# smritip/real-time-audio-sync

Hardware: AMD Instinct MI355X
Metric: aligned chroma frames/sec, batch=64 OTW c=500; path-index match vs CPU ref (higher is better)
Workload: dtype f64 arithmetic, f32 features in HBM

## Files before the change

include/rtsync.h:

```cpp
#ifndef RTSYNC_H
#define RTSYNC_H

#include <stddef.h>
#include <stdint.h>

#ifdef __cplusplus
extern "C" {
#endif

#define RTS_OK 0
#define RTS_ERR_INVALID (-1)
#define RTS_ERR_UNSUPPORTED (-2)
#define RTS_ERR_HIP (-3)
#define RTS_ERR_NO_DEVICE (-4)

#define RTS_F32 0
#define RTS_F64 1
#define RTS_I16 2

#define RTS_VARIANT_OTW 0
#define RTS_VARIANT_LIVENOTE 1
#define RTS_VARIANT_LIVENOTE_V2 2

#define RTS_COST_DOT 0
// ... 15 lines not shown
#define RTS_STATE_LEN 16
#define RTS_ST_T 0
#define RTS_ST_J 1
#define RTS_ST_DIRECTION 2
#define RTS_ST_PREVIOUS 3
#define RTS_ST_RUN_COUNT 4
#define RTS_ST_STATUS 5
#define RTS_ST_FIRST_INSERT 6
#define RTS_ST_N_PATH 7
#define RTS_ST_CONSUMED 8
#define RTS_ST_ROW_STRIPS 9
#define RTS_ST_COL_STRIPS 10
#define RTS_ST_CELLS_LO 11
#define RTS_ST_CELLS_HI 12
#define RTS_ST_PATH_TRUNCATED 13
#define RTS_ST_BAND_RECOMPUTES 15

const char *rts_last_error(void);
int rts_version(void);
int rts_device_count(void);

typedef struct rts_otw rts_otw;

int rts_otw_create(const void *ref_dev, int ref_dtype, int F, int N, int B, int c, int max_run_count,
                   int variant, int cost_kind, rts_otw **out);
int rts_otw_create_refs(const void *refs_dev, int ref_dtype, int F, long long n_ref_frames,
                        const long long *first_host, const int32_t *len_host, int B, int c, int max_run_count,
                        int variant, int cost_kind, rts_otw **out);
int rts_otw_destroy(rts_otw *h);
int rts_otw_reset(rts_otw *h, void *stream);

int rts_otw_restart(rts_otw *h, const uint8_t *mask_host, const long long *first_host, const int32_t *len_host,
                    void *stream);

int rts_otw_run(rts_otw *h, const void *live_dev, int live_dtype, int T_max, const int32_t *live_len_dev,
                int mode, void *stream);

int rts_otw_insert(rts_otw *h, const void *frames_dev, int frames_dtype, const uint8_t *active_dev,
                   void *stream);

int rts_otw_push(rts_otw *h, const void *frames_dev, int frames_dtype, int n_max, const int32_t *n_new_dev,
                 void *stream);

int rts_otw_recent(rts_otw *h, int M_max, double *out_dev , int32_t *len_dev ,
                   const uint8_t *mask_dev , void *stream);

int rts_otw_path_cost(rts_otw *h, int K, double *mean_dev , int32_t *n_dev ,
                      double *costs_dev , void *stream);

int rts_otw_read_state(rts_otw *h, int b, int32_t *state , void *stream);
int rts_otw_read_states(rts_otw *h, int32_t *states , void *stream);
int rts_otw_read_path(rts_otw *h, int b, int32_t *pairs, int cap_pairs, int *n, void *stream);
int rts_otw_read_bands(rts_otw *h, int b, double *row_band, double *col_band, void *stream);
int rts_otw_device_views(rts_otw *h, int32_t **path_dev, int *path_cap, int32_t **state_dev);
int rts_otw_set_dense(rts_otw *h, double *acc_dev, double *cost_dev, void *stream);
int rts_otw_replay_dense(rts_otw *h, const void *live_dev, int live_dtype, int T_max, const int32_t *live_len_dev,
                         double *acc_dev, double *cost_dev, void *stream);
int rts_otw_set_waves(rts_otw *h, int waves);
const char *rts_otw_kernel_name(const rts_otw *h);


int rts_dtw_workspace_bytes(int M, int N, int B, size_t *bytes);

int rts_dtw(const void *a_dev, int a_dtype, long long a_stride, const void *b_dev, int b_dtype,
            long long b_stride, int F, int M, int N, int B, double *cost_dev, double *acc_dev,
            int8_t *back_dev, int32_t *path_dev, int32_t *path_len_dev, void *ws_dev, size_t ws_bytes,
            void *stream);

int rts_dtw_paths_workspace_bytes(int M_max, int N_max, int B, size_t *bytes);

int rts_dtw_paths(const void *a_dev, int a_dtype, long long a_stride, const int32_t *a_len_dev, const void *b_dev,
                  int b_dtype, long long b_stride, const int32_t *b_len_dev, int F, int M_max, int N_max, int B,
                  int32_t *path_dev, int32_t *path_len_dev, double *total_dev, void *ws_dev, size_t ws_bytes,
                  void *stream);

int rts_dtw_subseq_paths_workspace_bytes(int M_max, int N_max, int B, size_t *bytes);

int rts_dtw_subseq_paths(const void *a_dev, int a_dtype, long long a_stride, const int32_t *a_len_dev,
                         const void *b_dev, int b_dtype, long long b_stride, const int32_t *b_len_dev,
                         int F, int M_max, int N_max, int B,
                         int32_t *path_dev, int32_t *path_len_dev, double *total_dev,
                         int32_t *start_dev, int32_t *end_dev, double *row_dev ,
                         void *ws_dev, size_t ws_bytes, void *stream);


int rts_locate(const void *queries_dev, int q_dtype, int M_max, const int32_t *q_len_dev, int B, const void *pool_dev,
               int pool_dtype, int F, long long n_pool_frames, const long long *piece_first_dev,
               const int32_t *piece_len_dev, int P, int cost_kind, double *cost_dev, int32_t *end_dev,
               int32_t *start_dev, double *row_dev, int32_t *rowstart_dev, void *stream);

typedef struct rts_chroma rts_chroma;

long long rts_chroma_num_frames(long long n_samples, int fft_len, int hop, int pad_left);

int rts_chroma_create(int fft_len, int hop, const double *window_host, const double *fb_host, rts_chroma **out);
int rts_chroma_destroy(rts_chroma *h);

int rts_chroma_frames(rts_chroma *h, const void *samples_dev, int sample_dtype, long long n_samples,
                      int pad_left, int n_frames, int normalize, void *chroma_out_dev, int out_dtype,
                      double *stft_out_dev, void *stream);

int rts_chroma_frames_batch(rts_chroma *h, const void *samples_dev, int sample_dtype, long long sample_stride,
                            const int32_t *n_samples_dev, int pad_left, int B, int n_frames_max,
                            const int32_t *n_frames_dev, int normalize, void *chroma_out_dev, int out_dtype,
                            void *stream);

// ... 85 lines not shown
```

real_time_audio_sync_amd/_native.py:

```python
import ctypes
import os

import torch

_HERE = os.path.dirname(os.path.abspath(__file__))
SO_PATH = os.environ.get("RTSYNC_LIB") or os.path.join(_HERE, "librtsync.so")

F32, F64, I16 = 0, 1, 2
VARIANT_OTW, VARIANT_LIVENOTE, VARIANT_LIVENOTE_V2 = 0, 1, 2
COST_DOT, COST_EUCLID = 0, 1
FEATURE_CHROMA, FEATURE_CHROMA_DIFF = 0, 1
DIR_NONE, DIR_BOTH, DIR_ROW, DIR_COLUMN = -1, 0, 1, 2
RUNNING, STOP_REF_END, LIVE_OVERFLOW, DEVICE_FAULT = 0, 1, 2, 3
MODE_INSERT_LOOP, MODE_SET_LIVE = 0, 1
STATE_LEN = 16
(ST_T, ST_J, ST_DIRECTION, ST_PREVIOUS, ST_RUN_COUNT, ST_STATUS, ST_FIRST_INSERT, ST_N_PATH, ST_CONSUMED,
 ST_ROW_STRIPS, ST_COL_STRIPS, ST_CELLS_LO, ST_CELLS_HI, ST_PATH_TRUNCATED) = range(14)
ST_BAND_RECOMPUTES = 15

EXPORTS = {}


class RtsyncError(RuntimeError):
    pass


def _load():
    if not os.path.exists(SO_PATH):
        raise ImportError(
            "librtsync.so is not built (%s). Run `python -c 'import __graft_entry__ as g; g.build()'` "
            "or `python real_time_audio_sync_amd/_build.py`. There is no CPU fallback." % SO_PATH)
    return ctypes.CDLL(SO_PATH)


lib = _load()

_vp, _i32, _pi32 = ctypes.c_void_p, ctypes.c_int, ctypes.POINTER(ctypes.c_int)


def _decl(name, restype, argtypes):
    fn = getattr(lib, name)
    fn.restype = restype
    fn.argtypes = argtypes
    EXPORTS[name] = fn
    return fn


_decl("rts_last_error", ctypes.c_char_p, [])
_decl("rts_version", _i32, [])
_decl("rts_device_count", _i32, [])
_decl("rts_otw_create", _i32, [_vp, _i32, _i32, _i32, _i32, _i32, _i32, _i32, _i32, ctypes.POINTER(_vp)])
_i64 = ctypes.c_longlong
_decl("rts_otw_create_refs", _i32, [_vp, _i32, _i32, _i64, _vp, _vp, _i32, _i32, _i32, _i32, _i32, ctypes.POINTER(_vp)])
_decl("rts_otw_destroy", _i32, [_vp])
_decl("rts_otw_reset", _i32, [_vp, _vp])
_decl("rts_otw_restart", _i32, [_vp, _vp, _vp, _vp, _vp])
_decl("rts_otw_run", _i32, [_vp, _vp, _i32, _i32, _vp, _i32, _vp])
_decl("rts_otw_insert", _i32, [_vp, _vp, _i32, _vp, _vp])
_decl("rts_otw_push", _i32, [_vp, _vp, _i32, _i32, _vp, _vp])
_decl("rts_otw_recent", _i32, [_vp, _i32, _vp, _vp, _vp, _vp])
_decl("rts_otw_path_cost", _i32, [_vp, _i32, _vp, _vp, _vp, _vp])
_decl("rts_otw_read_state", _i32, [_vp, _i32, _vp, _vp])
_decl("rts_otw_read_states", _i32, [_vp, _vp, _vp])
_decl("rts_otw_read_path", _i32, [_vp, _i32, _vp, _i32, _pi32, _vp])
_decl("rts_otw_read_bands", _i32, [_vp, _i32, _vp, _vp, _vp])
_decl("rts_otw_device_views", _i32, [_vp, ctypes.POINTER(_vp), _pi32, ctypes.POINTER(_vp)])
_decl("rts_otw_set_waves", _i32, [_vp, _i32])
_decl("rts_otw_set_dense", _i32, [_vp, _vp, _vp, _vp])
_decl("rts_otw_replay_dense", _i32, [_vp, _vp, _i32, _i32, _vp, _vp, _vp, _vp])
_decl("rts_otw_kernel_name", ctypes.c_char_p, [_vp])
_decl("rts_dtw_workspace_bytes", _i32, [_i32, _i32, _i32, ctypes.POINTER(ctypes.c_size_t)])
_decl("rts_dtw", _i32, [_vp, _i32, _i64, _vp, _i32, _i64, _i32, _i32, _i32, _i32, _vp, _vp, _vp, _vp, _vp, _vp,
                        ctypes.c_size_t, _vp])
_decl("rts_dtw_paths_workspace_bytes", _i32, [_i32, _i32, _i32, ctypes.POINTER(ctypes.c_size_t)])
_decl("rts_dtw_paths", _i32, [_vp, _i32, _i64, _vp, _vp, _i32, _i64, _vp, _i32, _i32, _i32, _i32, _vp, _vp, _vp, _vp,
                              ctypes.c_size_t, _vp])
_decl("rts_dtw_subseq_paths_workspace_bytes", _i32, [_i32, _i32, _i32, ctypes.POINTER(ctypes.c_size_t)])
_decl("rts_dtw_subseq_paths", _i32, [_vp, _i32, _i64, _vp, _vp, _i32, _i64, _vp, _i32, _i32, _i32, _i32, _vp, _vp, _vp, _vp,
                                     _vp, _vp, _vp, ctypes.c_size_t, _vp])
_decl("rts_locate", _i32, [_vp, _i32, _i32, _vp, _i32, _vp, _i32, _i32, _i64, _vp, _vp, _i32, _i32, _vp, _vp, _vp, _vp,
                           _vp, _vp])


_decl("rts_chroma_num_frames", _i64, [_i64, _i32, _i32, _i32])
_decl("rts_chroma_create", _i32, [_i32, _i32, _vp, _vp, ctypes.POINTER(_vp)])
_decl("rts_chroma_destroy", _i32, [_vp])
_decl("rts_chroma_frames", _i32, [_vp, _vp, _i32, _i64, _i32, _i32, _i32, _vp, _i32, _vp, _vp])
_decl("rts_chroma_frames_batch", _i32, [_vp, _vp, _i32, _i64, _vp, _i32, _i32, _i32, _vp, _i32, _vp, _i32, _vp])
_decl("rts_chroma_plan_info", _i32, [_vp, _pi32, _pi32])
_decl("rts_chroma_project", _i32, [_vp, _vp, _i32, _i32, _vp, _i32, _vp])
_decl("rts_chroma_diff", _i32, [_vp, _i32, _i32, _vp, _vp])


_decl("rts_resample_out_len", _i64, [_i64, _i32, _i32])
_decl("rts_resample_avail", _i64, [_i64, _i32, _i32, _i32])
_decl("rts_resample_create", _i32, [_i32, _i32, _vp, _i32, ctypes.POINTER(_vp)])
_decl("rts_resample_destroy", _i32, [_vp])
_decl("rts_resample_run", _i32, [_vp, _vp, _i32, _i64, _vp, _i32, _i32, _vp, _vp, _vp])


_decl("rts_wtw_create", _i32, [_vp, _i32, _i32, _i32, _i32, _i32, _i32, ctypes.POINTER(_vp)])
_decl("rts_wtw_create_refs", _i32, [_vp, _i32, _i64, _vp, _vp, _i32, _i32, _i32, _i32, ctypes.POINTER(_vp)])
_decl("rts_wtw_destroy", _i32, [_vp])
_decl("rts_wtw_reset", _i32, [_vp, _vp])
_decl("rts_wtw_restart", _i32, [_vp, _vp, _vp, _vp, _vp])
_decl("rts_wtw_push", _i32, [_vp, _vp, _i32, _i32, _vp, _i32, _vp])
_decl("rts_wtw_recent", _i32, [_vp, _i32, _vp, _vp, _vp, _vp])
_decl("rts_wtw_read_states", _i32, [_vp, _vp, _vp])
_decl("rts_wtw_read_path", _i32, [_vp, _i32, _vp, _i32, _pi32, _vp])
_decl("rts_wtw_read_last_d", _i32, [_vp, _i32, _vp, _vp])
_decl("rts_wtw_device_views", _i32, [_vp, ctypes.POINTER(_vp), _pi32, ctypes.POINTER(_vp)])
_decl("rts_wtw_state_view", _i32, [_vp, ctypes.POINTER(_vp)])
WTW_STATE_LEN = 8

_decl("rts_live_create", _i32, [_vp, _vp, _vp, _i32, _i32, ctypes.POINTER(_vp)])
_decl("rts_live_create_features", _i32, [_vp, _vp, _vp, _i32, _i32, _i32, ctypes.POINTER(_vp)])
_decl("rts_live_create_resampled", _i32, [_vp, _vp, _vp, _i32, _i32, _i32, _vp, ctypes.POINTER(_vp)])
_decl("rts_live_columns_view", _i32, [_vp, ctypes.POINTER(_vp), _pi32, _pi32, ctypes.POINTER(_vp)])
# ... 43 lines not shown
```

real_time_audio_sync_amd/csrc/otw.hip:

```cpp
#include <hip/hip_runtime.h>
#include <math.h>
#include <stddef.h>
#include <stdint.h>
#include <stdlib.h>
#include <string.h>
#include <type_traits>

#include "common.h"
#include "cost.h"

namespace rts {

constexpr int kF = 12;
constexpr int kFetch = 8;

struct OtwArgs {
    const void *ref;
    const void *live;
    const int32_t *live_len;
    int32_t *state;
    int32_t *path;
    double *bands;
    long long live_stride;
    int N, c, max_run_count, variant, cost_kind, mode;
// ... 2058 lines not shown
    const int32_t *state, *path, *hist_len;
    const double *hist;
    const void *ref;
    const long long *ref_first;
    const int32_t *ref_len;
    int N, path_cap, hist_stride, ref_f64, euclid, K;
    double *mean, *costs;
    int32_t *n_out;
};
__global__ void __launch_bounds__(256) otw_path_cost_kernel(PathCostArgs a) {
    __shared__ double cost_s[256];
    const int b = blockIdx.x, k = threadIdx.x;
    const double qnan = __longlong_as_double(0x7ff8000000000000LL);
    const int Nb = a.ref_len ? a.ref_len[b] : a.N;
    int points = a.state[(size_t)b * RTS_STATE_LEN + RTS_ST_N_PATH];
    points = points > a.path_cap ? a.path_cap : (points < 0 ? 0 : points);
    if (!a.hist) points = 0;
    const int n = points < a.K ? points : a.K;
    int frames = a.hist ? a.hist_len[b] : 0;
    frames = frames > a.hist_stride ? a.hist_stride : frames;
    if (k < a.K) {
        double cost = qnan;
        if (k < n) {
            const int2 p = reinterpret_cast<const int2 *>(a.path)[(size_t)b * a.path_cap + (points - n + k)];
            if (p.x >= 0 && p.x < frames && p.y >= 0 && p.y < Nb) {
                OtwEnv e;
                e.live = a.hist;
                e.live_f64 = 1;
                e.live_base = (long long)b * a.hist_stride * kF;
                e.ref_f64 = a.ref_f64;
                e.ref = a.ref_first ? static_cast<const char *>(a.ref) + a.ref_first[b] * (long long)kF * (a.ref_f64 ? 8 : 4)
                                    : a.ref;
                double lf[kF], rf[kF];
                otw_live_frame(e, p.x, lf);
                otw_ref_frame(e, p.y, rf);
                cost = cell_cost(lf, rf, a.euclid);
            }
        }
        cost_s[k] = cost;
        if (a.costs) a.costs[(size_t)b * a.K + k] = cost;
    }
    __syncthreads();
    if (k == 0) {
        double sum = 0.0;
        for (int i = 0; i < n; i++) sum = sum + cost_s[i];
        a.mean[b] = n > 0 ? sum / (double)n : qnan;
        a.n_out[b] = n;
        __threadfence_system();
    }
}

}

struct rts_otw {
    const void *ref;
    int ref_dtype, F, N, B, c, max_run_count, variant, cost_kind;
    int W, waves, path_cap;
    int hist_stride;
    int32_t *state;
    int32_t *path;
    double *bands;
    double *hist;
    rts::RefTable refs;
    int32_t *hist_len;
    long long *debug;
    double *dense_acc, *dense_cost;
    int spec;
    int device;
    int cus;
    int tp_from;
    const void *attr_fn[8];
    int src_kind;
    int run_dtype, run_T, run_mode;
    int32_t *rp_state, *rp_path;
    double *rp_bands;
};

namespace rts {

static int ensure_lds_attr(rts_otw *h, const void *fn, size_t smem) {
    for (int k = 0; k < 8; k++)
        if (h->attr_fn[k] == fn) return RTS_OK;
    RTS_HIP(hipFuncSetAttribute(fn, hipFuncAttributeMaxDynamicSharedMemorySize, (int)smem));
    for (int k = 0; k < 8; k++)
        if (!h->attr_fn[k]) {
            h->attr_fn[k] = fn;
            break;
        }
    return RTS_OK;
}

template <int W, int NW, bool DENSE, typename RT, bool SPEC>
static int launch_advance_d(rts_otw *h, const OtwArgs &args, int B, hipStream_t s) {
    using LdsT = OtwLds<W, RT>;
    const size_t smem = SPEC ? ((offsetof(LdsT, refw) + 15) & ~(size_t)15) + sizeof(OtwSpecLds<W>)
                             : (kHasLiveRing<RT> ? sizeof(LdsT) : ((offsetof(LdsT, refw) + 15) & ~(size_t)15));
    const int rc = ensure_lds_attr(h, reinterpret_cast<const void *>(&otw_advance_kernel<W, NW, DENSE, RT, SPEC>), smem);
    if (rc != RTS_OK) return rc;
    hipLaunchKernelGGL((otw_advance_kernel<W, NW, DENSE, RT, SPEC>), dim3(B), dim3(64 * NW), smem, s, args);
    RTS_HIP(hipGetLastError());
    return RTS_OK;
}

template <int W, int NW>
static int launch_advance(rts_otw *h, const OtwArgs &args, int B, hipStream_t s) {
    if constexpr (W >= 1024) {
        if (args.dense_acc) return launch_advance_d<W, 8, true, LiveFromGlobal, false>(h, args, B, s);
        if constexpr (NW >= 8) {
            if (args.spec) return launch_advance_d<W, NW, false, LiveFromGlobal, true>(h, args, B, s);
        }
        return set_error(RTS_ERR_UNSUPPORTED, "band widths above 500 (c=%d) run only on the pipelined 8-wave kernel", h->c);
    } else {
        if (args.dense_acc) return launch_advance_d<W, NW, true, double, false>(h, args, B, s);
        const bool f32 = !args.ref_f64 && !args.live_f64;
        if constexpr (NW >= 8) {
            if (args.spec) {
                if (B >= h->tp_from * h->cus && B > 0) return launch_advance_d<W, NW, false, LiveFromGlobalLean, true>(h, args, B, s);
                if (f32) return launch_advance_d<W, NW, false, float, true>(h, args, B, s);
                return (B <= h->cus) ? launch_advance_d<W, NW, false, double, true>(h, args, B, s)
                                     : launch_advance_d<W, NW, false, LiveFromGlobal, true>(h, args, B, s);
            }
        }
        return f32 ? launch_advance_d<W, NW, false, float, false>(h, args, B, s)
                   : launch_advance_d<W, NW, false, double, false>(h, args, B, s);
    }
}

template <int W>
static int launch_w(rts_otw *h, const OtwArgs &args, int B, int waves, hipStream_t s) {
    switch (waves) {
        case 1: return launch_advance<W, 1>(h, args, B, s);
        case 2: return launch_advance<W, 2>(h, args, B, s);
        case 4: return launch_advance<W, 4>(h, args, B, s);
        case 8: return launch_advance<W, 8>(h, args, B, s);
    }
    return set_error(RTS_ERR_INVALID, "waves must be 1, 2, 4 or 8 (got %d)", waves);
}

static int launch(rts_otw *h, const OtwArgs &args, hipStream_t s) {
    if ((uintptr_t)args.live & 15) return set_error(RTS_ERR_INVALID, "live features must be 16-byte aligned");
    switch (h->W) {
        case 64: return launch_w<64>(h, args, h->B, h->waves, s);
        case 128: return launch_w<128>(h, args, h->B, h->waves, s);
        case 256: return launch_w<256>(h, args, h->B, h->waves, s);
        case 512: return launch_w<512>(h, args, h->B, h->waves, s);
        case 1024: return launch_w<1024>(h, args, h->B, h->waves, s);
        case 2048: return launch_w<2048>(h, args, h->B, h->waves, s);
    }
    return set_error(RTS_ERR_UNSUPPORTED, "no kernel for window %d", h->W);
}

static OtwArgs base_args(const rts_otw *h) {
    OtwArgs a;
    memset(&a, 0, sizeof(a));
    a.ref = h->ref;
    a.state = h->state;
    a.path = h->path;
    a.bands = h->bands;
    a.N = h->N;
    a.c = h->c;
    a.max_run_count = h->max_run_count;
    a.variant = h->variant;
    a.cost_kind = h->cost_kind;
    a.path_cap = h->path_cap;
    a.live_cap = 2 * h->N;
    a.ref_first = h->refs.first;
    a.ref_len = h->refs.len;
    a.ref_f64 = h->ref_dtype == RTS_F64;
    a.debug = h->debug;
    a.spec = h->spec;
    a.dense_acc = h->dense_acc;
    a.dense_cost = h->dense_cost;
    return a;
}

static OtwArgs hist_args(const rts_otw *h) {
    OtwArgs a = base_args(h);
    a.live = h->hist;
    a.live_len = h->hist_len;
    a.live_stride = h->hist_stride;
    a.live_f64 = 1;
    a.mode = RTS_MODE_INSERT_LOOP;
    return a;
}

static int begin_append(rts_otw *h) {
    if (!h->hist) {
        RTS_HIP(hipMalloc((void **)&h->hist, sizeof(double) * kF * (size_t)h->hist_stride * h->B));
    }
    h->src_kind = (h->src_kind == 0 || h->src_kind == 2) ? 2 : 3;
    return RTS_OK;
}

static void fill_dense(const rts_otw *h, double *acc, double *cost, const RestartSel *sel, hipStream_t s) {
    const long long per = (long long)2 * h->N * h->N;
    const double sentinel = (h->variant == RTS_VARIANT_OTW) ? 1e10 : (double)INFINITY;
    if (sel) {
        hipLaunchKernelGGL(otw_fill_sel_kernel, dim3(64, sel->n), dim3(256), 0, s, *sel, acc, per, sentinel);
        hipLaunchKernelGGL(otw_fill_sel_kernel, dim3(64, sel->n), dim3(256), 0, s, *sel, cost, per, -1.0);
    } else {
        hipLaunchKernelGGL(otw_fill_kernel, dim3(2048), dim3(256), 0, s, acc, h->B * per, sentinel);
        hipLaunchKernelGGL(otw_fill_kernel, dim3(2048), dim3(256), 0, s, cost, h->B * per, -1.0);
    }
}

struct OtwKnobs {
    int spec, tp_from;
};
static OtwKnobs otw_knobs() {
    const char *sp = getenv("RTS_OTW_SPEC"), *tp = getenv("RTS_OTW_TP_FROM");
    return {sp ? (atoi(sp) != 0) : 1, tp ? atoi(tp) : 2};
}

static int otw_create(const void *ref_dev, int ref_dtype, int F, int N, int B, int c, int max_run_count, int variant,
                      int cost_kind, const long long *first_host, const int32_t *len_host, rts_otw **out) {
    if (F < 1) return set_error(RTS_ERR_INVALID, "F must be >= 1 (got %d)", F);
    if (F != kF) return set_error(RTS_ERR_UNSUPPORTED, "F must be 12 chroma bins (got %d)", F);
    if (N < 1 || B < 1) return set_error(RTS_ERR_INVALID, "N and B must be >= 1 (got N=%d B=%d)", N, B);
    if (ref_dtype != RTS_F32 && ref_dtype != RTS_F64) return set_error(RTS_ERR_INVALID, "bad ref_dtype %d", ref_dtype);
    if (c < 1) return set_error(RTS_ERR_INVALID, "c must be >= 1 (got %d)", c);
    if (c > 2036)
        return set_error(RTS_ERR_UNSUPPORTED, "band width c=%d exceeds the 2036 cells the LDS-resident kernel holds", c);
    if (max_run_count < 1) return set_error(RTS_ERR_INVALID, "max_run_count must be >= 1");
    if (variant < RTS_VARIANT_OTW || variant > RTS_VARIANT_LIVENOTE_V2)
        return set_error(RTS_ERR_INVALID, "bad variant %d", variant);
    if (cost_kind != RTS_COST_DOT && cost_kind != RTS_COST_EUCLID)
        return set_error(RTS_ERR_INVALID, "bad cost_kind %d", cost_kind);
    if ((long long)N * 3 + 8 > 0x3fffffffLL) return set_error(RTS_ERR_INVALID, "N too large");

    rts_otw *h = (rts_otw *)calloc(1, sizeof(rts_otw));
    if (!h) return set_error(RTS_ERR_INVALID, "out of host memory");
    h->ref = ref_dev;
    h->ref_dtype = ref_dtype;
    h->F = F;
    h->N = N;
    h->B = B;
    h->c = c;
    h->max_run_count = max_run_count;
    h->variant = variant;
    h->cost_kind = cost_kind;
    h->W = 64;
    while (h->W < c + 12) h->W *= 2;
    h->waves = 8;
    const OtwKnobs knobs = otw_knobs();
    h->spec = knobs.spec;
    h->tp_from = knobs.tp_from;
    h->hist_stride = 2 * N;
    h->path_cap = 3 * N + 8;
    hipError_t e;
    if ((e = hipGetDevice(&h->device)) != hipSuccess ||
        (e = hipDeviceGetAttribute(&h->cus, hipDeviceAttributeMultiprocessorCount, h->device)) != hipSuccess) {
        free(h);
        return set_error(RTS_ERR_HIP, "hipGetDevice failed: %s", hipGetErrorString(e));
    }
    if ((e = hipMalloc((void **)&h->state, sizeof(int32_t) * RTS_STATE_LEN * (size_t)B)) != hipSuccess ||
        (e = hipMalloc((void **)&h->path, sizeof(int32_t) * 2 * (size_t)h->path_cap * B)) != hipSuccess ||
        (e = hipMalloc((void **)&h->bands, sizeof(double) * 2 * (size_t)(c + 1) * B)) != hipSuccess ||
        (e = hipMalloc((void **)&h->hist_len, sizeof(int32_t) * (size_t)B)) != hipSuccess ||
        (first_host && (e = ref_table_upload(&h->refs, first_host, len_host, B)) != hipSuccess)) {
        rts_otw_destroy(h);
        return set_error(RTS_ERR_HIP, "hipMalloc failed: %s", hipGetErrorString(e));
    }
    int rc = rts_otw_reset(h, nullptr);
    if (rc != RTS_OK) {
        rts_otw_destroy(h);
        return rc;
    }
    hipLaunchKernelGGL(otw_fill_kernel, dim3(64), dim3(256), 0, nullptr, h->bands, (long long)2 * (c + 1) * B,
                       __builtin_nan(""));
    if ((e = hipGetLastError()) != hipSuccess) {
        rts_otw_destroy(h);
        return set_error(RTS_ERR_HIP, "launch of the band fill failed: %s", hipGetErrorString(e));
    }
    if ((e = hipStreamSynchronize(nullptr)) != hipSuccess) {
        rts_otw_destroy(h);
        return set_error(RTS_ERR_HIP, "hipStreamSynchronize failed: %s", hipGetErrorString(e));
    }
    *out = h;
    return RTS_OK;
}

int otw_batch(const rts_otw *h) { return h->B; }

}

extern "C" {

int rts_otw_create(const void *ref_dev, int ref_dtype, int F, int N, int B, int c, int max_run_count,
                   int variant, int cost_kind, rts_otw **out) {
    using namespace rts;
    if (!out) return set_error(RTS_ERR_INVALID, "out is NULL");
    *out = nullptr;
    if (!ref_dev) return set_error(RTS_ERR_INVALID, "ref_dev is NULL");
    return otw_create(ref_dev, ref_dtype, F, N, B, c, max_run_count, variant, cost_kind, nullptr, nullptr, out);
}

int rts_otw_create_refs(const void *refs_dev, int ref_dtype, int F, long long n_ref_frames,
                        const long long *first_host, const int32_t *len_host, int B, int c, int max_run_count,
                        int variant, int cost_kind, rts_otw **out) {
    using namespace rts;
    if (!out) return set_error(RTS_ERR_INVALID, "out is NULL");
    *out = nullptr;
    if (!refs_dev) return set_error(RTS_ERR_INVALID, "refs_dev is NULL");
    if (!first_host || !len_host) return set_error(RTS_ERR_INVALID, "first_host / len_host is NULL");
    if (B < 1) return set_error(RTS_ERR_INVALID, "B must be >= 1 (got %d)", B);
    const int n_max = ref_ranges_check(B, nullptr, first_host, len_host, n_ref_frames, 0, nullptr);
    if (n_max < 0) return n_max;
    const int rc = otw_create(refs_dev, ref_dtype, F, n_max, B, c, max_run_count, variant, cost_kind, first_host, len_host, out);
    if (rc == RTS_OK) (*out)->refs.n_frames = n_ref_frames;
    return rc;
}

int rts_otw_destroy(rts_otw *h) {
    if (!h) return RTS_OK;
    if (h->state) (void)hipFree(h->state);
    if (h->path) (void)hipFree(h->path);
    if (h->bands) (void)hipFree(h->bands);
    if (h->hist) (void)hipFree(h->hist);
    if (h->hist_len) (void)hipFree(h->hist_len);
    rts::ref_table_free(&h->refs);
    if (h->rp_state) (void)hipFree(h->rp_state);
    if (h->rp_path) (void)hipFree(h->rp_path);
    if (h->rp_bands) (void)hipFree(h->rp_bands);
    free(h);
    return RTS_OK;
}

int rts_otw_reset(rts_otw *h, void *stream) {
    using namespace rts;
    if (!h) return set_error(RTS_ERR_INVALID, "handle is NULL");
    if (int rc = check_device(h->device, "handle"); rc != RTS_OK) return rc;
    hipStream_t s = (hipStream_t)stream;
    h->src_kind = 0;
    hipLaunchKernelGGL(otw_reset_kernel, dim3((h->B + 63) / 64), dim3(64), 0, s, h->state, h->B, h->variant);
    RTS_HIP(hipGetLastError());
    RTS_HIP(hipMemsetAsync(h->hist_len, 0, sizeof(int32_t) * (size_t)h->B, s));
    if (h->dense_acc) {
        fill_dense(h, h->dense_acc, h->dense_cost, nullptr, s);
        RTS_HIP(hipGetLastError());
    }
    return RTS_OK;
}

int rts_otw_restart(rts_otw *h, const uint8_t *mask_host, const long long *first_host, const int32_t *len_host,
                    void *stream) {
    using namespace rts;
    if (!h) return set_error(RTS_ERR_INVALID, "handle is NULL");
    if (!mask_host) return set_error(RTS_ERR_INVALID, "mask_host is NULL");
    if (int rc = restart_check(h->B, mask_host, first_host, len_host, h->refs.first ? h->refs.n_frames : -1, h->N, "N_max");
        rc != RTS_OK)
        return rc;
    if (int rc = check_device(h->device, "handle"); rc != RTS_OK) return rc;
    hipStream_t s = (hipStream_t)stream;
    RestartSel sel;
    for (int pos = 0; restart_next_chunk(h->B, mask_host, first_host, len_host, &pos, &sel) > 0;) {
        hipLaunchKernelGGL(otw_restart_kernel, dim3(sel.n), dim3(64), 0, s, sel, h->state, h->hist_len, h->bands,
                           2 * (h->c + 1), h->refs.first, h->refs.len, h->variant);
        if (h->dense_acc) fill_dense(h, h->dense_acc, h->dense_cost, &sel, s);
        RTS_HIP(hipGetLastError());
    }
    return RTS_OK;
}

int rts_otw_set_dense(rts_otw *h, double *acc_dev, double *cost_dev, void *stream) {
    using namespace rts;
    if (!h) return set_error(RTS_ERR_INVALID, "handle is NULL");
    if (h->refs.first)
        return set_error(RTS_ERR_UNSUPPORTED, "the dense mirror is not available on a handle with per-stream references");
    if ((acc_dev == nullptr) != (cost_dev == nullptr))
        return set_error(RTS_ERR_INVALID, "acc_dev and cost_dev must both be given or both be NULL");
    h->dense_acc = acc_dev;
    h->dense_cost = cost_dev;
    return rts_otw_reset(h, stream);
}

int rts_otw_replay_dense(rts_otw *h, const void *live_dev, int live_dtype, int T_max, const int32_t *live_len_dev,
                         double *acc_dev, double *cost_dev, void *stream) {
    using namespace rts;
    if (!h) return set_error(RTS_ERR_INVALID, "handle is NULL");
    if (h->refs.first)
        return set_error(RTS_ERR_UNSUPPORTED, "the dense replay is not available on a handle with per-stream references");
    if (!acc_dev || !cost_dev) return set_error(RTS_ERR_INVALID, "acc_dev / cost_dev is NULL");
    if (int rc = check_device(h->device, "handle"); rc != RTS_OK) return rc;
    if (h->src_kind == 3)
        return set_error(RTS_ERR_UNSUPPORTED, "rts_otw_insert / rts_otw_push after rts_otw_run without a reset: nothing to replay from");
    if (h->src_kind == 1) {
        if (!live_dev || !live_len_dev)
            return set_error(RTS_ERR_INVALID, "the handle's frames came from rts_otw_run: pass that call's live_dev / live_len_dev again");
        if (live_dtype != RTS_F32 && live_dtype != RTS_F64) return set_error(RTS_ERR_INVALID, "bad live_dtype %d", live_dtype);
        if (live_dtype != h->run_dtype || T_max != h->run_T)
            return set_error(RTS_ERR_INVALID, "live_dtype / T_max differ from the rts_otw_run being replayed (%d / %d then)", h->run_dtype, h->run_T);
    } else if (live_dev) {
        return set_error(RTS_ERR_INVALID, "the handle's frames came through rts_otw_insert / rts_otw_push (or it is fresh): live_dev must be NULL");
    }
    hipStream_t s = (hipStream_t)stream;
    fill_dense(h, acc_dev, cost_dev, nullptr, s);
    RTS_HIP(hipGetLastError());
    if (h->src_kind == 0) return RTS_OK;
    if (!h->rp_state) {
        hipError_t e;
        if ((e = hipMalloc((void **)&h->rp_state, sizeof(int32_t) * RTS_STATE_LEN * (size_t)h->B)) != hipSuccess ||
            (e = hipMalloc((void **)&h->rp_path, sizeof(int32_t) * 2 * (size_t)h->path_cap * h->B)) != hipSuccess ||
            (e = hipMalloc((void **)&h->rp_bands, sizeof(double) * 2 * (size_t)(h->c + 1) * h->B)) != hipSuccess) {
            if (h->rp_state) (void)hipFree(h->rp_state);
            if (h->rp_path) (void)hipFree(h->rp_path);
            h->rp_state = h->rp_path = nullptr;
            return set_error(RTS_ERR_HIP, "hipMalloc failed: %s", hipGetErrorString(e));
        }
    }
    hipLaunchKernelGGL(otw_reset_kernel, dim3((h->B + 63) / 64), dim3(64), 0, s, h->rp_state, h->B, h->variant);
    OtwArgs a = h->src_kind == 1 ? base_args(h) : hist_args(h);
    a.state = h->rp_state;
    a.path = h->rp_path;
    a.bands = h->rp_bands;
    a.dense_acc = acc_dev;
    a.dense_cost = cost_dev;
    if (h->src_kind == 1) {
        a.live = live_dev;
        a.live_len = live_len_dev;
        a.live_stride = T_max;
        a.live_f64 = live_dtype == RTS_F64;
        a.mode = h->run_mode;
        a.clamp_len = 1;
    }
    int rc = launch(h, a, s);
    if (rc != RTS_OK) return rc;
    RTS_HIP(hipStreamSynchronize(s));
    return RTS_OK;
}

int rts_otw_set_waves(rts_otw *h, int waves) {
    using namespace rts;
    if (!h) return set_error(RTS_ERR_INVALID, "handle is NULL");
    if (waves != 1 && waves != 2 && waves != 4 && waves != 8)
        return set_error(RTS_ERR_INVALID, "waves must be 1, 2, 4 or 8 (got %d)", waves);
    h->waves = waves;
    return RTS_OK;
}

const char *rts_otw_kernel_name(const rts_otw *) { return "otw_advance_kernel"; }

int rts_otw_run(rts_otw *h, const void *live_dev, int live_dtype, int T_max, const int32_t *live_len_dev,
                int mode, void *stream) {
    using namespace rts;
    if (!h) return set_error(RTS_ERR_INVALID, "handle is NULL");
    if (!live_dev || !live_len_dev) return set_error(RTS_ERR_INVALID, "live_dev / live_len_dev is NULL");
    if (live_dtype != RTS_F32 && live_dtype != RTS_F64) return set_error(RTS_ERR_INVALID, "bad live_dtype %d", live_dtype);
    if (T_max < 0) return set_error(RTS_ERR_INVALID, "T_max < 0");
    if (mode != RTS_MODE_INSERT_LOOP && mode != RTS_MODE_SET_LIVE) return set_error(RTS_ERR_INVALID, "bad mode %d", mode);
    hipStream_t s = (hipStream_t)stream;
    int rc = rts_otw_reset(h, stream);
    if (rc != RTS_OK) return rc;
    OtwArgs a = base_args(h);
    a.live = live_dev;
    a.live_len = live_len_dev;
    a.live_stride = T_max;
    a.live_f64 = live_dtype == RTS_F64;
    a.mode = mode;
    a.clamp_len = 1;
    h->src_kind = 1;
    h->run_dtype = live_dtype;
    h->run_T = T_max;
    h->run_mode = mode;
    return launch(h, a, s);
}

int rts_otw_insert(rts_otw *h, const void *frames_dev, int frames_dtype, const uint8_t *active_dev, void *stream) {
    using namespace rts;
    if (!h) return set_error(RTS_ERR_INVALID, "handle is NULL");
    if (!frames_dev) return set_error(RTS_ERR_INVALID, "frames_dev is NULL");
    if (frames_dtype != RTS_F32 && frames_dtype != RTS_F64) return set_error(RTS_ERR_INVALID, "bad frames_dtype %d", frames_dtype);
    hipStream_t s = (hipStream_t)stream;
    if (int rc = check_device(h->device, "handle"); rc != RTS_OK) return rc;
    if (int rc = begin_append(h); rc != RTS_OK) return rc;
    hipLaunchKernelGGL(otw_append_kernel, dim3(h->B), dim3(64), 0, s, h->hist, h->hist_len, frames_dev,
                       frames_dtype == RTS_F64, active_dev, h->B, h->hist_stride);
    RTS_HIP(hipGetLastError());
    return launch(h, hist_args(h), s);
}

int rts_otw_push(rts_otw *h, const void *frames_dev, int frames_dtype, int n_max, const int32_t *n_new_dev,
                 void *stream) {
    using namespace rts;
    if (!h) return set_error(RTS_ERR_INVALID, "handle is NULL");
    if (n_max < 0) return set_error(RTS_ERR_INVALID, "n_max < 0");
    if (n_max == 0) return RTS_OK;
    if (!frames_dev) return set_error(RTS_ERR_INVALID, "frames_dev is NULL");
    if (frames_dtype != RTS_F32 && frames_dtype != RTS_F64) return set_error(RTS_ERR_INVALID, "bad frames_dtype %d", frames_dtype);
    hipStream_t s = (hipStream_t)stream;
    if (int rc = check_device(h->device, "handle"); rc != RTS_OK) return rc;
    if (int rc = begin_append(h); rc != RTS_OK) return rc;
    hipLaunchKernelGGL(otw_append_many_kernel, dim3(h->B), dim3(128), 0, s, h->hist, h->hist_len, frames_dev,
                       frames_dtype == RTS_F64, n_new_dev, n_max, n_max, h->B, h->hist_stride);
    RTS_HIP(hipGetLastError());
    return launch(h, hist_args(h), s);
}

static int refuse_run_frames(const rts_otw *h, const char *what) {
    if (h->src_kind == 1 || h->src_kind == 3)
        return rts::set_error(RTS_ERR_UNSUPPORTED, "%s: the handle has consumed an rts_otw_run since its last reset, whose frames "
                                                   "are the caller's memory and not in the handle's history", what);
    return RTS_OK;
}

int rts_otw_recent(rts_otw *h, int M_max, double *out_dev, int32_t *len_dev, const uint8_t *mask_dev, void *stream) {
    using namespace rts;
    if (!h) return set_error(RTS_ERR_INVALID, "handle is NULL");
    if (!out_dev) return set_error(RTS_ERR_INVALID, "out_dev is NULL");
    if (!len_dev) return set_error(RTS_ERR_INVALID, "len_dev is NULL");
    if (M_max < 1) return set_error(RTS_ERR_INVALID, "M_max must be >= 1 (got %d)", M_max);
    if (M_max > 256) return set_error(RTS_ERR_UNSUPPORTED, "M_max = %d exceeds the 256 frames rts_locate takes", M_max);
    if (int rc = refuse_run_frames(h, "rts_otw_recent"); rc != RTS_OK) return rc;
    if (int rc = check_device(h->device, "handle"); rc != RTS_OK) return rc;
    hipLaunchKernelGGL(otw_recent_kernel, dim3(h->B), dim3(256), 0, (hipStream_t)stream, h->hist, h->hist_len, h->hist_stride,
                       h->N, h->refs.len, M_max, out_dev, len_dev, mask_dev);
    RTS_HIP(hipGetLastError());
    return RTS_OK;
}

int rts_otw_path_cost(rts_otw *h, int K, double *mean_dev, int32_t *n_dev, double *costs_dev, void *stream) {
    using namespace rts;
    if (!h) return set_error(RTS_ERR_INVALID, "handle is NULL");
    if (!mean_dev) return set_error(RTS_ERR_INVALID, "mean_dev is NULL");
    if (!n_dev) return set_error(RTS_ERR_INVALID, "n_dev is NULL");
    if (K < 1 || K > 256) return set_error(RTS_ERR_INVALID, "K must be in [1, 256] (got %d)", K);
    if (int rc = refuse_run_frames(h, "rts_otw_path_cost"); rc != RTS_OK) return rc;
    if (int rc = check_device(h->device, "handle"); rc != RTS_OK) return rc;
    PathCostArgs a;
    a.state = h->state;
    a.path = h->path;
    a.hist_len = h->hist_len;
    a.hist = h->hist;
    a.ref = h->ref;
    a.ref_first = h->refs.first;
    a.ref_len = h->refs.len;
    a.N = h->N;
    a.path_cap = h->path_cap;
    a.hist_stride = h->hist_stride;
    a.ref_f64 = h->ref_dtype == RTS_F64;
    a.euclid = h->cost_kind == RTS_COST_EUCLID;
    a.K = K;
    a.mean = mean_dev;
    a.costs = costs_dev;
    a.n_out = n_dev;
    hipLaunchKernelGGL(otw_path_cost_kernel, dim3(h->B), dim3(64 * ((K + 63) / 64)), 0, (hipStream_t)stream, a);
    RTS_HIP(hipGetLastError());
    return RTS_OK;
}

int rts_otw_read_states(rts_otw *h, int32_t *states, void *stream) {
    using namespace rts;
    if (!h || !states) return set_error(RTS_ERR_INVALID, "NULL argument");
    hipStream_t s = (hipStream_t)stream;
    RTS_HIP(hipMemcpyAsync(states, h->state, sizeof(int32_t) * RTS_STATE_LEN * (size_t)h->B, hipMemcpyDeviceToHost, s));
    RTS_HIP(hipStreamSynchronize(s));
    for (int b = 0; b < h->B; b++) states[b * RTS_STATE_LEN + 14] = 0;
    return RTS_OK;
}

int rts_otw_read_state(rts_otw *h, int b, int32_t *state, void *stream) {
    using namespace rts;
    if (!h || !state) return set_error(RTS_ERR_INVALID, "NULL argument");
    if (b < 0 || b >= h->B) return set_error(RTS_ERR_INVALID, "stream index %d out of range [0, %d)", b, h->B);
    hipStream_t s = (hipStream_t)stream;
    RTS_HIP(hipMemcpyAsync(state, h->state + (size_t)b * RTS_STATE_LEN, sizeof(int32_t) * RTS_STATE_LEN,
                           hipMemcpyDeviceToHost, s));
    RTS_HIP(hipStreamSynchronize(s));
    state[14] = 0;
    return RTS_OK;
}

int rts_otw_read_path(rts_otw *h, int b, int32_t *pairs, int cap_pairs, int *n, void *stream) {
    using namespace rts;
    if (!h || !n) return set_error(RTS_ERR_INVALID, "NULL argument");
    return read_path(h->state, RTS_STATE_LEN, RTS_ST_N_PATH, h->path, h->path_cap, b, h->B, pairs, cap_pairs, n,
                     (hipStream_t)stream);
}

int rts_otw_read_bands(rts_otw *h, int b, double *row_band, double *col_band, void *stream) {
    using namespace rts;
    if (!h || !row_band || !col_band) return set_error(RTS_ERR_INVALID, "NULL argument");
    if (b < 0 || b >= h->B) return set_error(RTS_ERR_INVALID, "stream index %d out of range [0, %d)", b, h->B);
    hipStream_t s = (hipStream_t)stream;
    const double *bb = h->bands + (size_t)b * 2 * (h->c + 1);
    RTS_HIP(hipMemcpyAsync(row_band, bb, sizeof(double) * (h->c + 1), hipMemcpyDeviceToHost, s));
    RTS_HIP(hipMemcpyAsync(col_band, bb + (h->c + 1), sizeof(double) * (h->c + 1), hipMemcpyDeviceToHost, s));
    RTS_HIP(hipStreamSynchronize(s));
    return RTS_OK;
}

#ifdef RTS_OTW_STAMPS
int rts_otw_set_debug(rts_otw *h, long long *debug_dev) {
    if (!h) return rts::set_error(RTS_ERR_INVALID, "handle is NULL");
    h->debug = debug_dev;
    return RTS_OK;
}
int rts_otw_stamp_level(void) { return RTS_OTW_STAMPS; }
int rts_otw_debug_words(void) { return (RTS_OTW_STAMPS == 2) ? 64 : 16; }
#endif

int rts_otw_device_views(rts_otw *h, int32_t **path_dev, int *path_cap, int32_t **state_dev) {
    using namespace rts;
    if (!h) return set_error(RTS_ERR_INVALID, "handle is NULL");
    if (path_dev) *path_dev = h->path;
    if (path_cap) *path_cap = h->path_cap;
    if (state_dev) *state_dev = h->state;
    return RTS_OK;
}

}
```

real_time_audio_sync_amd/otw_batch.py:

```python
import ctypes

import numpy as np
import torch

from . import _native as nat
from ._handle import _BatchedHandle, _concat_refs

_VARIANTS = {"otw": nat.VARIANT_OTW, "livenote": nat.VARIANT_LIVENOTE, "livenote_v2": nat.VARIANT_LIVENOTE_V2}


def _np_dtype_code(dt):
    if dt == torch.float32:
        return nat.F32
    if dt == torch.float64:
        return nat.F64
    raise TypeError("feature tensors must be float32 or float64, got %s" % dt)


def frames_tensor(x, device, dtype=None):
    if isinstance(x, np.ndarray):
        x = torch.from_numpy(np.ascontiguousarray(x))
    if dtype is not None:
        x = x.to(dtype)
    return x.to(device).t().contiguous()
# ... 97 lines not shown
        assert frames_dev.is_contiguous() and frames_dev.shape[0] == self.B and frames_dev.shape[2] == 12
        self._version += 1
        nat.check(nat.lib.rts_otw_push(self._h, frames_dev.data_ptr(), _np_dtype_code(frames_dev.dtype),
                                       int(frames_dev.shape[1]), n_new_dev.data_ptr() if n_new_dev is not None else None,
                                       self._stream()))

    @_on_device
    def reset(self):
        self._version += 1
        self._keep = None
        nat.check(nat.lib.rts_otw_reset(self._h, self._stream()))

    def restart(self, streams, refs=None, offsets=None):
        super().restart(streams, refs, offsets)
        self._version += 1

    @_on_device
    def path_cost(self, K=64, want_costs=False):
        K = int(K)
        mean = torch.empty(self.B, dtype=torch.float64, device=self.device)
        n = torch.empty(self.B, dtype=torch.int32, device=self.device)
        costs = torch.empty((self.B, max(K, 0)), dtype=torch.float64, device=self.device) if want_costs else None
        nat.check(nat.lib.rts_otw_path_cost(self._h, K, mean.data_ptr(), n.data_ptr(),
                                            costs.data_ptr() if want_costs else None, self._stream()))
        return (mean, n, costs) if want_costs else (mean, n)

    @_on_device
    def states(self):
        out = np.zeros((self.B, nat.STATE_LEN), dtype=np.int32)
        nat.check(nat.lib.rts_otw_read_states(self._h, out.ctypes.data, self._stream()))
        return out

    def state(self, b=0):
        s = self.states()[b]
        cells = (int(np.uint32(s[nat.ST_CELLS_HI])) << 32) | int(np.uint32(s[nat.ST_CELLS_LO]))
        return dict(t=int(s[nat.ST_T]), j=int(s[nat.ST_J]), direction=int(s[nat.ST_DIRECTION]),
                    previous=int(s[nat.ST_PREVIOUS]), run_count=int(s[nat.ST_RUN_COUNT]),
                    status=int(s[nat.ST_STATUS]), first_insert=int(s[nat.ST_FIRST_INSERT]),
                    n_path=int(s[nat.ST_N_PATH]), consumed=int(s[nat.ST_CONSUMED]),
                    row_strips=int(s[nat.ST_ROW_STRIPS]), col_strips=int(s[nat.ST_COL_STRIPS]), cells=cells,
                    path_truncated=int(s[nat.ST_PATH_TRUNCATED]), band_recomputes=int(s[nat.ST_BAND_RECOMPUTES]))

    def paths(self):
        return [self.path(b) for b in range(self.B)]

    @_on_device
    def bands(self, b=0):
        rb = np.empty(self.c + 1)
        cb = np.empty(self.c + 1)
        nat.check(nat.lib.rts_otw_read_bands(self._h, b, rb.ctypes.data, cb.ctypes.data, self._stream()))
        return rb, cb

    @_on_device
    def enable_dense(self):
        if self.ref_lens is not None:
            nat.check(nat.lib.rts_otw_set_dense(self._h, None, None, self._stream()))
        self.dense_acc = torch.empty((self.B, 2 * self.N, self.N), dtype=torch.float64, device=self.device)
        self.dense_cost = torch.empty((self.B, 2 * self.N, self.N), dtype=torch.float64, device=self.device)
        nat.check(nat.lib.rts_otw_set_dense(self._h, self.dense_acc.data_ptr(), self.dense_cost.data_ptr(),
                                            self._stream()))
        return self.dense_acc, self.dense_cost

    @_on_device
    def replay_dense(self):
        if self.ref_lens is not None:
            nat.check(nat.lib.rts_otw_replay_dense(self._h, None, nat.F64, 0, None, None, None, self._stream()))
        acc = torch.empty((self.B, 2 * self.N, self.N), dtype=torch.float64, device=self.device)
        cost = torch.empty((self.B, 2 * self.N, self.N), dtype=torch.float64, device=self.device)
        if self._keep is not None:
            lv, ln = self._keep
            nat.check(nat.lib.rts_otw_replay_dense(self._h, lv.data_ptr(), _np_dtype_code(lv.dtype), int(lv.shape[1]),
                                                   ln.data_ptr(), acc.data_ptr(), cost.data_ptr(), self._stream()))
        else:
            nat.check(nat.lib.rts_otw_replay_dense(self._h, None, nat.F64, 0, None, acc.data_ptr(), cost.data_ptr(),
                                                   self._stream()))
        return acc, cost

    @_on_device
    def set_waves(self, waves):
        nat.check(nat.lib.rts_otw_set_waves(self._h, int(waves)))

    @property
    def kernel_name(self):
        return nat.lib.rts_otw_kernel_name(self._h).decode()
```

Measured before the change: 34.11 million.

## Add wavefront band-fill kernel for the initial c×c OTW window

Adds a new kernel that, on the first insert of a batch with at least c frames, computes the whole initial c×c DTW block in parallel. It uses an anti-diagonal wavefront across waves with LDS handoff, writes the row and column bands, the path and the state, then lets the existing sequential OTW kernel continue from that state. This replaces the serial step-by-step startup, which has little parallelism, with a parallel fill. The cost is an extra launch, a large shared-memory footprint, a one-time exactness risk in the reconstructed path (every step marked as diagonal), and an env knob that is on by default.

```diff
diff --git a/include/rtsync.h b/include/rtsync.h
--- a/include/rtsync.h
+++ b/include/rtsync.h
@@ -91,6 +91,7 @@
 int rts_otw_read_states(rts_otw *h, int32_t *states , void *stream);
 int rts_otw_read_path(rts_otw *h, int b, int32_t *pairs, int cap_pairs, int *n, void *stream);
 int rts_otw_read_bands(rts_otw *h, int b, double *row_band, double *col_band, void *stream);
+int rts_otw_read_fill(rts_otw *h, int32_t *took , void *stream);
 int rts_otw_device_views(rts_otw *h, int32_t **path_dev, int *path_cap, int32_t **state_dev);
 int rts_otw_set_dense(rts_otw *h, double *acc_dev, double *cost_dev, void *stream);
 int rts_otw_replay_dense(rts_otw *h, const void *live_dev, int live_dtype, int T_max, const int32_t *live_len_dev,
diff --git a/real_time_audio_sync_amd/_native.py b/real_time_audio_sync_amd/_native.py
--- a/real_time_audio_sync_amd/_native.py
+++ b/real_time_audio_sync_amd/_native.py
@@ -64,6 +64,7 @@
 _decl("rts_otw_read_states", _i32, [_vp, _vp, _vp])
 _decl("rts_otw_read_path", _i32, [_vp, _i32, _vp, _i32, _pi32, _vp])
 _decl("rts_otw_read_bands", _i32, [_vp, _i32, _vp, _vp, _vp])
+_decl("rts_otw_read_fill", _i32, [_vp, _vp, _vp])
 _decl("rts_otw_device_views", _i32, [_vp, ctypes.POINTER(_vp), _pi32, ctypes.POINTER(_vp)])
 _decl("rts_otw_set_waves", _i32, [_vp, _i32])
 _decl("rts_otw_set_dense", _i32, [_vp, _vp, _vp, _vp])
diff --git a/real_time_audio_sync_amd/csrc/otw.hip b/real_time_audio_sync_amd/csrc/otw.hip
--- a/real_time_audio_sync_amd/csrc/otw.hip
+++ b/real_time_audio_sync_amd/csrc/otw.hip
@@ -2134,6 +2134,8 @@
 
 }
 
+#include "otw_fill.h"
+
 struct rts_otw {
     const void *ref;
     int ref_dtype, F, N, B, c, max_run_count, variant, cost_kind;
@@ -2151,6 +2153,9 @@
     int device;
     int cus;
     int tp_from;
+    int fill;
+    int fill_last;
+    int32_t *fill_took;
     const void *attr_fn[8];
     int src_kind;
     int run_dtype, run_T, run_mode;
@@ -2219,8 +2224,15 @@
     return set_error(RTS_ERR_INVALID, "waves must be 1, 2, 4 or 8 (got %d)", waves);
 }
 
-static int launch(rts_otw *h, const OtwArgs &args, hipStream_t s) {
+static int launch(rts_otw *h, const OtwArgs &args, hipStream_t s, int max_new) {
     if ((uintptr_t)args.live & 15) return set_error(RTS_ERR_INVALID, "live features must be 16-byte aligned");
+    const bool fill = h->fill && max_new >= h->c && h->c >= 2 && h->W <= 512 && !args.dense_acc;
+    if (args.state == h->state) h->fill_last = fill;
+    if (fill) {
+        const dim3 block(otw_fill_threads(h->c));
+        hipLaunchKernelGGL(otw_bandfill_kernel, dim3(h->B), block, 0, s, args, h->fill_took);
+        RTS_HIP(hipGetLastError());
+    }
     switch (h->W) {
         case 64: return launch_w<64>(h, args, h->B, h->waves, s);
         case 128: return launch_w<128>(h, args, h->B, h->waves, s);
@@ -2287,11 +2299,11 @@
 }
 
 struct OtwKnobs {
-    int spec, tp_from;
+    int spec, tp_from, fill;
 };
 static OtwKnobs otw_knobs() {
-    const char *sp = getenv("RTS_OTW_SPEC"), *tp = getenv("RTS_OTW_TP_FROM");
-    return {sp ? (atoi(sp) != 0) : 1, tp ? atoi(tp) : 2};
+    const char *sp = getenv("RTS_OTW_SPEC"), *tp = getenv("RTS_OTW_TP_FROM"), *fl = getenv("RTS_OTW_FILL");
+    return {sp ? (atoi(sp) != 0) : 1, tp ? atoi(tp) : 2, fl ? (atoi(fl) != 0) : 1};
 }
 
 static int otw_create(const void *ref_dev, int ref_dtype, int F, int N, int B, int c, int max_run_count, int variant,
@@ -2327,6 +2339,7 @@
     const OtwKnobs knobs = otw_knobs();
     h->spec = knobs.spec;
     h->tp_from = knobs.tp_from;
+    h->fill = knobs.fill;
     h->hist_stride = 2 * N;
     h->path_cap = 3 * N + 8;
     hipError_t e;
@@ -2339,6 +2352,7 @@
         (e = hipMalloc((void **)&h->path, sizeof(int32_t) * 2 * (size_t)h->path_cap * B)) != hipSuccess ||
         (e = hipMalloc((void **)&h->bands, sizeof(double) * 2 * (size_t)(c + 1) * B)) != hipSuccess ||
         (e = hipMalloc((void **)&h->hist_len, sizeof(int32_t) * (size_t)B)) != hipSuccess ||
+        (e = hipMalloc((void **)&h->fill_took, sizeof(int32_t) * (size_t)B)) != hipSuccess ||
         (first_host && (e = ref_table_upload(&h->refs, first_host, len_host, B)) != hipSuccess)) {
         rts_otw_destroy(h);
         return set_error(RTS_ERR_HIP, "hipMalloc failed: %s", hipGetErrorString(e));
@@ -2400,6 +2414,7 @@
     if (h->bands) (void)hipFree(h->bands);
     if (h->hist) (void)hipFree(h->hist);
     if (h->hist_len) (void)hipFree(h->hist_len);
+    if (h->fill_took) (void)hipFree(h->fill_took);
     rts::ref_table_free(&h->refs);
     if (h->rp_state) (void)hipFree(h->rp_state);
     if (h->rp_path) (void)hipFree(h->rp_path);
@@ -2505,7 +2520,7 @@
         a.mode = h->run_mode;
         a.clamp_len = 1;
     }
-    int rc = launch(h, a, s);
+    int rc = launch(h, a, s, 0);
     if (rc != RTS_OK) return rc;
     RTS_HIP(hipStreamSynchronize(s));
     return RTS_OK;
@@ -2544,7 +2559,7 @@
     h->run_dtype = live_dtype;
     h->run_T = T_max;
     h->run_mode = mode;
-    return launch(h, a, s);
+    return launch(h, a, s, T_max);
 }
 
 int rts_otw_insert(rts_otw *h, const void *frames_dev, int frames_dtype, const uint8_t *active_dev, void *stream) {
@@ -2558,7 +2573,7 @@
     hipLaunchKernelGGL(otw_append_kernel, dim3(h->B), dim3(64), 0, s, h->hist, h->hist_len, frames_dev,
                        frames_dtype == RTS_F64, active_dev, h->B, h->hist_stride);
     RTS_HIP(hipGetLastError());
-    return launch(h, hist_args(h), s);
+    return launch(h, hist_args(h), s, 1);
 }
 
 int rts_otw_push(rts_otw *h, const void *frames_dev, int frames_dtype, int n_max, const int32_t *n_new_dev,
@@ -2575,7 +2590,7 @@
     hipLaunchKernelGGL(otw_append_many_kernel, dim3(h->B), dim3(128), 0, s, h->hist, h->hist_len, frames_dev,
                        frames_dtype == RTS_F64, n_new_dev, n_max, n_max, h->B, h->hist_stride);
     RTS_HIP(hipGetLastError());
-    return launch(h, hist_args(h), s);
+    return launch(h, hist_args(h), s, n_max);
 }
 
 static int refuse_run_frames(const rts_otw *h, const char *what) {
@@ -2659,6 +2674,19 @@
                      (hipStream_t)stream);
 }
 
+int rts_otw_read_fill(rts_otw *h, int32_t *took, void *stream) {
+    using namespace rts;
+    if (!h || !took) return set_error(RTS_ERR_INVALID, "NULL argument");
+    if (!h->fill_last) {
+        memset(took, 0, sizeof(int32_t) * (size_t)h->B);
+        return RTS_OK;
+    }
+    hipStream_t s = (hipStream_t)stream;
+    RTS_HIP(hipMemcpyAsync(took, h->fill_took, sizeof(int32_t) * (size_t)h->B, hipMemcpyDeviceToHost, s));
+    RTS_HIP(hipStreamSynchronize(s));
+    return RTS_OK;
+}
+
 int rts_otw_read_bands(rts_otw *h, int b, double *row_band, double *col_band, void *stream) {
     using namespace rts;
     if (!h || !row_band || !col_band) return set_error(RTS_ERR_INVALID, "NULL argument");
diff --git a/real_time_audio_sync_amd/csrc/otw_fill.h b/real_time_audio_sync_amd/csrc/otw_fill.h
--- /dev/null
+++ b/real_time_audio_sync_amd/csrc/otw_fill.h
@@ -0,0 +1,220 @@
+#pragma once
+
+namespace rts {
+
+constexpr int kFillMaxC = 500;
+
+__device__ __forceinline__ bool otw_fill_eligible(const OtwArgs &a, int b, int nthreads, int &live_len_out, int &N_out) {
+    const int32_t *st = a.state + (size_t)b * RTS_STATE_LEN;
+    int live_len = a.live_len[b];
+    if (a.clamp_len && live_len > (int)a.live_stride) live_len = (int)a.live_stride;
+    const int N = a.ref_first ? a.ref_len[b] : a.N;
+    live_len_out = live_len;
+    N_out = N;
+    const int c = a.c;
+    const int need = c + ((a.mode == RTS_MODE_SET_LIVE) ? 1 : 0);
+    return st[RTS_ST_FIRST_INSERT] == 1 && st[RTS_ST_STATUS] == RTS_RUNNING && st[RTS_ST_CONSUMED] == 0 &&
+           st[RTS_ST_N_PATH] == 0 && c >= 2 && c <= kFillMaxC && c <= nthreads && live_len >= need && N >= c &&
+           a.path_cap >= c && a.dense_acc == nullptr;
+}
+
+constexpr int kFillPad = 64, kFillCols = kFillPad + 512 + kFillPad;
+constexpr int kFillRows = 2;
+
+__host__ __device__ constexpr int otw_fill_threads(int c) { return 64 * (((c + kFillRows - 1) / kFillRows + 63) / 64); }
+
+__global__ void __launch_bounds__(64 * ((kFillMaxC / kFillRows + 63) / 64)) otw_bandfill_kernel(OtwArgs a, int32_t *took) {
+    constexpr int R = kFillRows;
+    __shared__ double refs[kF][kFillCols];
+    __shared__ double hand_v[2][8], hand_cv[2][8];
+    __shared__ int hand_ci[2][8];
+    int2 *pts = reinterpret_cast<int2 *>(&refs[0][0]);
+
+    const int tid = threadIdx.x, lane = tid & 63;
+    const int wave = __builtin_amdgcn_readfirstlane(tid >> 6);
+    const int nw = (int)blockDim.x >> 6;
+    const int b = blockIdx.x, c = a.c, p = tid;
+    int live_len, N;
+    const bool ok = otw_fill_eligible(a, b, R * (int)blockDim.x, live_len, N);
+    if (tid == 0) took[b] = ok ? 1 : 0;
+    if (!ok) return;
+
+    const double inf = INFINITY;
+    const bool set_live = a.mode == RTS_MODE_SET_LIVE;
+    const int euclid = a.cost_kind == RTS_COST_EUCLID;
+    OtwEnv e;
+    e.b = b;
+    e.lane = lane;
+    e.live = a.live;
+    e.live_f64 = a.live_f64;
+    e.live_base = (long long)b * a.live_stride * kF;
+    const void *ref = a.ref_first ? static_cast<const void *>(static_cast<const char *>(a.ref) +
+                                                              a.ref_first[b] * (long long)kF * (a.ref_f64 ? 8 : 4))
+                                  : a.ref;
+    double lf[R][kF];
+#pragma unroll
+    for (int r = 0; r < R; r++) otw_live_frame(e, (R * p + r < c) ? R * p + r : c - 1, lf[r]);
+    for (int idx = tid; idx < kF * kFillCols; idx += (int)blockDim.x) (&refs[0][0])[idx] = 0.0;
+    __syncthreads();
+    for (int idx = tid; idx < c * kF; idx += (int)blockDim.x) {
+        const int fr = idx / kF, f = idx % kF;
+        refs[f][kFillPad + fr] = otw_load_feat(ref, a.ref_f64, (long long)fr * kF + f);
+    }
+    __syncthreads();
+
+    double *bb = a.bands + (size_t)b * 2 * (c + 1);
+    double val[R], rmin[R], dgp = inf, cv = inf, d00 = 0.0;
+    int ridx[R], px[R], py[R], ci = 0x7fffffff;
+#pragma unroll
+    for (int r = 0; r < R; r++) {
+        val[r] = inf;
+        rmin[r] = inf;
+        ridx[r] = 0x7fffffff;
+        px[r] = py[r] = 0;
+    }
+    const int P = (c + R - 1) / R;
+    const int d_lo = 64 * wave, d_hi = 64 * wave + 63 + c - 1;
+    const double *rp = &refs[0][kFillPad + d_lo - p];
+    for (int d = 0; d <= P + c - 2; d++) {
+        if (d >= d_lo && d <= d_hi) {
+            const int j = d - p;
+            double hin_v = inf, hin_cv = inf;
+            int hin_ci = 0x7fffffff;
+            if (wave > 0) {
+                const int s = (d - 1) & 1;
+                hin_v = hand_v[s][wave - 1];
+                hin_cv = hand_cv[s][wave - 1];
+                hin_ci = hand_ci[s][wave - 1];
+            }
+            double rf[kF];
+#pragma unroll
+            for (int f = 0; f < kF; f++) rf[f] = rp[f * kFillCols];
+            rp += 1;
+            double dc[R];
+#pragma unroll
+            for (int r = 0; r < R; r++) dc[r] = cell_cost(lf[r], rf, euclid);
+            const double up0 = wave_shift_up(val[R - 1], hin_v);
+            double cvr = wave_shift_up(cv, hin_cv);
+            int cir = __builtin_amdgcn_update_dpp(hin_ci, ci, 0x138, 0xf, 0xf, false);
+            const bool warm = d < d_lo + 63, outside = j < 0;
+            const bool on_diag = d >= (R + 1) * d_lo && d <= (R + 1) * (d_lo + 63) + R - 1;
+            const bool last_col = d >= d_lo + c - 1;
+            double up = up0, dg = dgp;
+#pragma unroll
+            for (int r = 0; r < R; r++) {
+                const int i = R * p + r;
+                double nv = vmin(vmin(up + dc[r], dg + 2 * dc[r]), val[r] + dc[r]);
+                if (warm) nv = outside ? inf : nv;
+                if (r == 0 && d == 0) {
+                    if (p == 0) {
+                        nv = dc[0];
+                        d00 = nv;
+                    }
+                }
+                const bool rless = nv < rmin[r];
+                rmin[r] = vmin(rmin[r], nv);
+                ridx[r] = rless ? j : ridx[r];
+                const bool cless = nv < cvr;
+                cvr = vmin(cvr, nv);
+                cir = cless ? i : cir;
+                if (on_diag) {
+                    if (j == i) {
+                        const bool rw = rmin[r] < cvr;
+                        px[r] = rw ? i : cir;
+                        py[r] = rw ? ridx[r] : i;
+                    }
+                }
+                if (wave == nw - 1) {
+                    if (i == c - 1 && j >= 0 && j < c) bb[1 + j] = nv;
+                }
+                if (last_col) {
+                    if (j == c - 1 && i < c) bb[(c + 1) + 1 + i] = nv;
+                }
+                dg = val[r];
+                up = nv;
+                val[r] = nv;
+            }
+            dgp = up0;
+            cv = cvr;
+            ci = cir;
+            if (wave < nw - 1) {
+                if (lane == 63) {
+                    hand_v[d & 1][wave] = val[R - 1];
+                    hand_cv[d & 1][wave] = cv;
+                    hand_ci[d & 1][wave] = ci;
+                }
+            }
+        }
+        lds_barrier();
+    }
+
+    const bool filt = a.variant == RTS_VARIANT_LIVENOTE_V2;
+    int2 *path = reinterpret_cast<int2 *>(a.path) + (size_t)b * a.path_cap;
+    const int sl = set_live ? 1 : 0;
+#pragma unroll
+    for (int r = 0; r < R; r++) {
+        const int i = R * p + r;
+        if (!filt) {
+            if (i >= 1 && i < c) path[i - 1 + sl] = make_int2(px[r], py[r]);
+        } else if (i < c) {
+            pts[i] = make_int2(px[r], py[r]);
+        }
+    }
+    __syncthreads();
+    if (tid == 0) {
+        int32_t *st = a.state + (size_t)b * RTS_STATE_LEN;
+        const bool deferred = set_live && a.variant != RTS_VARIANT_OTW;
+        int run_count = st[RTS_ST_RUN_COUNT], prev = st[RTS_ST_PREVIOUS], pend = -2, n_path = 0, last_x = -1, last_y = -1;
+        for (int t = set_live ? 0 : 1; t < c; t++) {
+            if (t > 0 && deferred && pend != -2) {
+                run_count = (pend == prev) ? run_count + 1 : 1;
+                if (pend != RTS_DIR_BOTH) prev = pend;
+                pend = -2;
+            }
+            int x = 0, y = 0;
+            if (t == 0) {
+                x = (d00 != d00) ? 0x7fffffff : 0;
+                if (!filt) path[0] = make_int2(x, y);
+            } else if (filt) {
+                x = pts[t].x;
+                y = pts[t].y;
+            }
+            if (filt && (n_path == 0 || (x > last_x && y >= last_y))) {
+                path[n_path] = make_int2(x, y);
+                n_path += 1;
+                last_x = x;
+                last_y = y;
+            } else if (!filt) {
+                n_path += 1;
+            }
+            const int nd = RTS_DIR_BOTH;
+            if (deferred) {
+                pend = nd;
+            } else {
+                run_count = (nd == prev) ? run_count + 1 : 1;
+                if (nd != RTS_DIR_BOTH) prev = nd;
+            }
+        }
+        const double qnan = __longlong_as_double(0x7ff8000000000000LL);
+        bb[0] = qnan;
+        bb[c + 1] = qnan;
+        st[RTS_ST_T] = c - 1;
+        st[RTS_ST_J] = c - 1;
+        st[RTS_ST_DIRECTION] = RTS_DIR_BOTH;
+        st[RTS_ST_PREVIOUS] = prev;
+        st[RTS_ST_RUN_COUNT] = run_count;
+        st[RTS_ST_STATUS] = RTS_RUNNING;
+        st[RTS_ST_FIRST_INSERT] = 0;
+        st[RTS_ST_N_PATH] = n_path;
+        st[RTS_ST_CONSUMED] = c;
+        st[RTS_ST_ROW_STRIPS] = c - 1;
+        st[RTS_ST_COL_STRIPS] = c - 1;
+        st[RTS_ST_CELLS_LO] = c * c;
+        st[RTS_ST_CELLS_HI] = 0;
+        st[RTS_ST_PATH_TRUNCATED] = 0;
+        st[14] = pend;
+        st[RTS_ST_BAND_RECOMPUTES] = 0;
+    }
+}
+
+}
diff --git a/real_time_audio_sync_amd/otw_batch.py b/real_time_audio_sync_amd/otw_batch.py
--- a/real_time_audio_sync_amd/otw_batch.py
+++ b/real_time_audio_sync_amd/otw_batch.py
@@ -173,6 +173,12 @@
         return rb, cb
 
     @_on_device
+    def fill_taken(self):
+        out = np.zeros(self.B, dtype=np.int32)
+        nat.check(nat.lib.rts_otw_read_fill(self._h, out.ctypes.data, self._stream()))
+        return out
+
+    @_on_device
     def enable_dense(self):
         if self.ref_lens is not None:
             nat.check(nat.lib.rts_otw_set_dense(self._h, None, None, self._stream()))
```

After: 36.14 million (median of 6 runs). 5.9% higher.
